# cafferychen777/flashdeconv

Hardware: AMD Instinct MI355X
Metric: spots/sec to convergence (1M x 2000 x 30) (higher is better)
Workload: dtype f64

## Files before the change

### flashdeconv_amd/_lib.py

```python
import ctypes
import os
import threading

import numpy as np

_HERE = os.path.dirname(os.path.abspath(__file__))
LIB_PATH = os.path.join(_HERE, "libfdx.so")

c_int = ctypes.c_int
c_i32 = ctypes.c_int32
c_i64 = ctypes.c_int64
c_double = ctypes.c_double
c_void_p = ctypes.c_void_p
c_size_t = ctypes.c_size_t
p_double = ctypes.POINTER(ctypes.c_double)
p_i64 = ctypes.POINTER(ctypes.c_int64)
p_i32 = ctypes.POINTER(ctypes.c_int32)


class FdxError(RuntimeError):
    """A libfdx call failed (message from fdx_last_error())."""


class SolveInfo(ctypes.Structure):
# ... 97 lines not shown
    "fdx_graph_shard_knn_dev": (c_int, [c_void_p, c_i64, c_i32, c_i32, c_i32, p_i64, c_i32, c_void_p, ctypes.POINTER(c_void_p)]),
    "fdx_graph_shard_status": (c_int, [c_void_p, p_i64, p_i64, p_i32, p_i32]),
    "fdx_graph_row_indices": (c_int, [c_void_p, c_i64, p_i32, c_i32, p_i32]),
    "fdx_graph_halo_info": (c_int, [c_void_p, p_i64, p_i32, p_i32]),
    "fdx_graph_send_indices_dev": (c_int, [c_void_p, c_void_p, c_void_p]),
    "fdx_prepare_dev": (c_int, [c_void_p, c_i32, c_i64, c_i32, c_i64, c_void_p, p_double, c_i32, p_i32, p_double, p_double,
                                c_i32, c_i32, c_i32, c_void_p, c_i64, c_void_p, p_double, p_double, c_void_p]),
    "fdx_init_beta_dev": (c_int, [c_void_p, c_i64, c_i64, c_i32, c_void_p]),
    "fdx_bcd_sweep_dev": (c_int, [c_void_p, c_void_p, c_i64, c_void_p, c_void_p, c_void_p, c_i64, c_i32, c_double, c_double,
                                  c_double, c_i32, c_void_p, c_void_p, c_void_p]),
    "fdx_bcd_fold_dev": (c_int, [c_void_p, c_void_p, c_i32, c_void_p]),
    "fdx_objective_partials_dev": (c_int, [c_void_p, c_void_p, c_i64, c_void_p, c_i64, c_void_p, c_i32, p_double, c_void_p]),
    "fdx_spot_diagnostics_dev": (c_int, [c_void_p, c_void_p, c_i64, c_void_p, c_i64, c_void_p, c_i32, c_i32, c_void_p, c_void_p,
                                         c_void_p]),
    "fdx_normalize_dev": (c_int, [c_void_p, c_i64, c_i64, c_i32, c_void_p, c_void_p, c_void_p]),
    "fdx_gene_moments_dev": (c_int, [c_void_p, c_i32, c_i64, c_i32, c_i64, p_double, p_double, c_void_p]),
    "fdx_gather_columns_dev": (c_int, [c_void_p, c_i32, c_i64, c_i32, c_i64, p_i32, c_i32, c_void_p, c_void_p]),
    "fdx_version": (c_int, []),
    "fdx_env_reload": (c_int, []),
    "fdx_env_switch": (ctypes.c_char_p, [c_i32, ctypes.POINTER(ctypes.c_char_p)]),
    "fdx_last_error": (ctypes.c_char_p, []),
    "fdx_device_count": (c_int, [ctypes.POINTER(c_int)]),
    "fdx_set_device": (c_int, [c_int]),
    "fdx_device_name": (c_int, [ctypes.c_char_p, c_int]),
    "fdx_malloc": (c_int, [ctypes.POINTER(c_void_p), c_size_t]),
    "fdx_free": (c_int, [c_void_p]),
    "fdx_trim": (c_int, []),
    "fdx_memcpy_h2d": (c_int, [c_void_p, c_void_p, c_size_t, c_void_p]),
    "fdx_memcpy_d2h": (c_int, [c_void_p, c_void_p, c_size_t, c_void_p]),
    "fdx_memset": (c_int, [c_void_p, c_int, c_size_t, c_void_p]),
# ... 451 lines not shown
```

### flashdeconv_amd/csrc/bcd_kernels.cpp

```cpp
#include <algorithm>

#include "bcd_device.h"

namespace fdx {

__global__ __launch_bounds__(256) void bcd_sweep_generic_kernel(BcdSweepArgs a, double* scratch, size_t sld) {
    const int lane = threadIdx.x & 63;
    const int wib = __builtin_amdgcn_readfirstlane(threadIdx.x >> 6);
    const int K = a.K;
    if (a.it > 0) {
        const double rc = fold_rel_change(a.stats + (size_t)(a.it - 1) * 128, lane);
        if (blockIdx.x == 0 && threadIdx.x == 0) a.rel_change[a.it - 1] = rc;
        if (rc < a.tol) return;
    }
    const int slice = xcd_remap(blockIdx.x, gridDim.x) * 4 + wib;
    if (slice >= a.n_slices) return;
    const int i = slice * 64 + lane;
    const bool active = i < a.n;
    const int ii = active ? i : a.n - 1;
    const size_t ld = (size_t)a.ld;
    const int w0 = a.slice_off[slice];
    const int w = a.slice_off[slice + 1] - w0;
    double* bb = scratch + (size_t)(slice * 64 + lane);
    const int* ell = a.ell + (size_t)w0 * 64 + lane;
// ... 310 lines not shown
        for (int A = 0; A < nblk; ++A)
            for (int B = A; B < nblk; ++B)
                hipLaunchKernelGGL(beta_quad_block_kernel, dim3(grid), dim3(256), 0, st, beta, ld, n, K, XtX, A * 4, B * 4, A == B ? 1.0 : 2.0,
                                   partials);
        FDX_CHECK_LAUNCH();
        return 0;
    }
#define FDX_BQ(T) case T: hipLaunchKernelGGL(beta_quad_kernel<T>, dim3(grid), dim3(256), 0, st, beta, ld, n, K, XtX, partials); break;
    switch (TT) { FDX_BQ(1) FDX_BQ(2) FDX_BQ(3) FDX_BQ(4) FDX_BQ(5) FDX_BQ(6) FDX_BQ(7) default: return fail(FDX_ERR_INVALID, "beta quad: K"); }
#undef FDX_BQ
    FDX_CHECK_LAUNCH();
    return 0;
}

int launch_bcd_objective_tiled(const BcdSweepArgs& a0, double* partials, hipStream_t st) {
    if (!a0.tiled || !sweep_instantiated(a0.K)) return 1;
    const int KC = a0.K < 8 ? a0.K : 8;
    if ((size_t)KC * (256 + a0.halo_max + 1) * sizeof(double) > 64 * 1024) return 1;
    BcdSweepArgs a = a0;
    a.objective = 1;
    a.rel_change = partials;
    a.it = 0;
    const bool hit = bcd_sweep_dispatch_part0(a, st) || bcd_sweep_dispatch_part1(a, st) || bcd_sweep_dispatch_part2(a, st) ||
                     bcd_sweep_dispatch_part3(a, st) || bcd_sweep_dispatch_part4(a, st) || bcd_sweep_dispatch_part5(a, st) ||
                     bcd_sweep_dispatch_part6(a, st) || bcd_sweep_dispatch_part7(a, st);
    if (!hit) return 1;
    FDX_CHECK_LAUNCH();
    return 0;
}

int launch_bcd_fold_last(const unsigned long long* stats, double* rel_change, int it, hipStream_t st) {
    hipLaunchKernelGGL(bcd_fold_last_kernel, dim3(1), dim3(64), 0, st, stats, rel_change, it);
    FDX_CHECK_LAUNCH();
// ... 5 lines not shown
```

### flashdeconv_amd/csrc/bcd_sweep_inst.cpp

```cpp
#include <algorithm>
#include <cstdlib>
#include "bcd_device.h"
#include "fdx_graph.h"

#ifndef FDX_PART
#error "compile with -DFDX_PART=<n> -DFDX_K_LO=<lo> -DFDX_K_HI=<hi>"
#endif

namespace fdx {

constexpr int sweep_chunk(int K) {
#ifdef FDX_KC_OVERRIDE
    return K < FDX_KC_OVERRIDE ? K : FDX_KC_OVERRIDE;
#endif
    return K < 8 ? K : K <= 29 ? 8 : K <= 33 ? 7 : K <= 37 ? 6 : K <= 41 ? 5 : K <= 45 ? 4 : K <= 49 ? 3 : K <= 51 ? 2 : K <= 64 ? 8 : K <= 72 ? 6 : K <= 88 ? 4 : K <= 96 ? 2 : 8;
}

template <int K, int KC>
__global__ __launch_bounds__(256) void bcd_sweep_kernel(
    const double* __restrict__ H, const double* __restrict__ XtX, const double* __restrict__ beta_in,
    double* __restrict__ beta_out, const int* __restrict__ ell_base, const int* __restrict__ slice_off,
    const int* __restrict__ deg, unsigned long long* __restrict__ stats, double* __restrict__ rel_change,
    const double lambda, const double rho, const double tol, const int ldh, const int ld_, const int n,
    const int n_slices, const int it) {
// ... 71 lines not shown
        atomicMax(s + 64 + slot, (unsigned long long)__double_as_longlong(amax));
    }
}

__device__ __forceinline__ const char __attribute__((address_space(1)))* plane_base(const double* p) {
    unsigned long long v = (unsigned long long)p;
    asm("" : "+s"(v));
    return (const char __attribute__((address_space(1)))*)v;
}

__device__ __forceinline__ unsigned lane_off(unsigned off) {
    asm("" : "+v"(off));
    return off;
}

#ifndef FDX_SWEEP_WPE
#define FDX_SWEEP_WPE 1
#endif
template <int K, int KC, bool OBJ, bool QUAD = true, bool INIT = false>
__global__ __launch_bounds__(256, ((OBJ && K > 40 && K <= 64) || (K > 64 && K <= 96)) ? 2 : (OBJ ? 1 : FDX_SWEEP_WPE)) void bcd_sweep_tiled_kernel(
    const double* __restrict__ H, const double* __restrict__ XtX, const double* __restrict__ beta_in,
    double* __restrict__ beta_out, const unsigned short* __restrict__ ell_local, const int* __restrict__ slice_off,
    const int* __restrict__ deg, const int* __restrict__ tile_halo, const int* __restrict__ tile_hcnt,
    unsigned long long* __restrict__ stats, double* __restrict__ rel_change, const double lambda, const double rho,
    const double tol, const int ldh, const int ld_, const int n, const int S, const int it,
    const int* __restrict__ tile_list, const double init_v, const int* __restrict__ send_head, const int4* __restrict__ send_ent,
    double* __restrict__ send_buf) {
    extern __shared__ __attribute__((aligned(16))) double lds[];
    const int tid = threadIdx.x;
    const int lane = tid & 63;
    const int tile = tile_list ? tile_list[xcd_remap(blockIdx.x, gridDim.x)] : xcd_remap(blockIdx.x, gridDim.x);
    const bool real = (tile * 256 + tid) < n;
    const int i = min(tile * 256 + tid, n - 1);
    const size_t ld = (size_t)ld_;
    const int slice = __builtin_amdgcn_readfirstlane(i >> 6);
    const int w0 = slice_off[slice];
    const int w = slice_off[slice + 1] - w0;
    const int Ht = tile_hcnt[tile];
    const int* halo = tile_halo + (size_t)tile * FDX_TILE_HALO_CAP;
    const int dg = deg[i];
    int hidx0 = halo[tid];
    if (!OBJ && it > 0) {
// ... 81 lines not shown
                if (!OBJ || QUAD) {
#pragma unroll
                    for (int j = 0; j + 1 < K; j += 2) {
                        r0 = fma(g[j], b[j], r0);
                        r1 = fma(g[j + 1], b[j + 1], r1);
                    }
                    if (K & 1) r0 = fma(g[K - 1], b[K - 1], r0);
                }
                const double gkk = (!OBJ || QUAD) ? g[k] : 0.0;
                const double old = b[k];
                if (OBJ) {
                    o_cross = fma(old, h, o_cross);
                    if (QUAD) o_quad = fma(old, r0 + r1, o_quad);
                    o_spat = fma(old, (double)dg * old - c[q], o_spat);
                    o_l1 += fabs(old);
                    asm volatile("" : "+v"(o_quad));
                } else {
                    const double res = (h - (r0 + r1) + gkk * old) + lam_eff * c[q];
                    const double den = gkk + lam_deg;
                    const double st = res > rho ? res - rho : (res < -rho ? res + rho : 0.0);
                    const double qv = fmax(0.0, st / den);
                    const double nw = (den > 1e-10) ? qv : 0.0;
                    dmax = fmax(dmax, fabs(nw - old));
                    amax = fmax(amax, fabs(old));
                    b[k] = nw;
                    __builtin_nontemporal_store(nw, (double __attribute__((address_space(1)))*)(plane_base(beta_out + k * ld) + lane_off(ioff)));
                }
            }
            if (kc + KC < K) {
#pragma unroll
                for (int t = 2 * q; t < 2 * q + 2; ++t) {
                    const int j = t < KC ? t : t - KC;
                    if (kc + KC + j < K) {
                        if (t < KC) { if (!INIT) hv[j] = PLANE_AT(beta_in + (kc + KC + j) * ld, hoff); }
                        else hreg[j] = __builtin_nontemporal_load(&PLANE_AT(H + (kc + KC + j) * (size_t)ldh, ioff));
                    }
                }
                __builtin_amdgcn_sched_barrier(0);
            }
        }
    }
    if (OBJ) {
        if (!real) { o_cross = o_quad = o_spat = o_l1 = 0.0; }
#pragma unroll
        for (int off = 32; off > 0; off >>= 1) {
            o_cross += __shfl_xor(o_cross, off, 64);
            o_quad += __shfl_xor(o_quad, off, 64);
            o_spat += __shfl_xor(o_spat, off, 64);
            o_l1 += __shfl_xor(o_l1, off, 64);
        }
        __syncthreads();
        if (lane == 0) { lds[(tid >> 6) * 4 + 0] = o_cross; lds[(tid >> 6) * 4 + 1] = o_quad; lds[(tid >> 6) * 4 + 2] = o_spat; lds[(tid >> 6) * 4 + 3] = o_l1; }
        __syncthreads();
        if (tid < 4) rel_change[(size_t)tile * 4 + tid] = ((lds[tid] + lds[4 + tid]) + lds[8 + tid]) + lds[12 + tid];
        return;
    }
    if (!OBJ && send_head != nullptr) {
// ... 15 lines not shown
        atomicMax(s + 64 + slot, (unsigned long long)__double_as_longlong(amax));
    }
}

template <int K>
static void launch_k(const BcdSweepArgs& a, hipStream_t st) {
    if (a.tiled) {
        constexpr int KC = sweep_chunk(K);
        const int S = 256 + a.halo_max + 1;
        const size_t lds = (size_t)KC * S * sizeof(double);
        if (lds <= 64 * 1024 && (long long)a.ld * 8 < (1LL << 32) && (long long)a.ldh * 8 < (1LL << 32)) {
            if (a.objective) {
                if constexpr (K > 64) {
                    hipLaunchKernelGGL((bcd_sweep_tiled_kernel<K, KC, true, false>), dim3(a.n_tiles), dim3(256), lds, st, a.H, a.XtX,
                                       a.beta_in, a.beta_out, a.ell_local, a.slice_off, a.deg, a.tile_halo, a.tile_hcnt,
                                       a.stats, a.rel_change, a.lambda, a.rho, a.tol, a.ldh, a.ld, a.n, S, a.it, nullptr, 0.0, a.send_head, a.send_ent, a.send_buf);
                } else {
                    hipLaunchKernelGGL((bcd_sweep_tiled_kernel<K, KC, true>), dim3(a.n_tiles), dim3(256), lds, st, a.H, a.XtX,
                                       a.beta_in, a.beta_out, a.ell_local, a.slice_off, a.deg, a.tile_halo, a.tile_hcnt,
                                       a.stats, a.rel_change, a.lambda, a.rho, a.tol, a.ldh, a.ld, a.n, S, a.it, nullptr, 0.0, a.send_head, a.send_ent, a.send_buf);
                }
            }
            else if (a.tile_list) {
                if (a.n_list > 0)
                    hipLaunchKernelGGL((bcd_sweep_tiled_kernel<K, KC, false>), dim3(a.n_list), dim3(256), lds, st, a.H, a.XtX,
                                       a.beta_in, a.beta_out, a.ell_local, a.slice_off, a.deg, a.tile_halo, a.tile_hcnt,
                                       a.stats, a.rel_change, a.lambda, a.rho, a.tol, a.ldh, a.ld, a.n, S, a.it, a.tile_list, 0.0, a.send_head, a.send_ent, a.send_buf);
            } else if (a.init_uniform != 0.0) {
                if constexpr (K <= 64) {
                    hipLaunchKernelGGL((bcd_sweep_tiled_kernel<K, KC, false, true, true>), dim3(a.n_tiles), dim3(256), lds, st, a.H, a.XtX,
                                       a.beta_in, a.beta_out, a.ell_local, a.slice_off, a.deg, a.tile_halo, a.tile_hcnt,
                                       a.stats, a.rel_change, a.lambda, a.rho, a.tol, a.ldh, a.ld, a.n, S, a.it, nullptr, a.init_uniform, a.send_head, a.send_ent, a.send_buf);
                }
            } else {
                hipLaunchKernelGGL((bcd_sweep_tiled_kernel<K, KC, false>), dim3(a.n_tiles), dim3(256), lds, st, a.H, a.XtX,
                                   a.beta_in, a.beta_out, a.ell_local, a.slice_off, a.deg, a.tile_halo, a.tile_hcnt,
                                   a.stats, a.rel_change, a.lambda, a.rho, a.tol, a.ldh, a.ld, a.n, S, a.it, nullptr, 0.0, a.send_head, a.send_ent, a.send_buf);
            }
            return;
        }
    }
    const int nblk = ceil_div(a.n_slices, 4);
    hipLaunchKernelGGL((bcd_sweep_kernel<K, sweep_chunk(K)>), dim3(nblk), dim3(256), 0, st, a.H, a.XtX, a.beta_in,
                       a.beta_out, a.ell, a.slice_off, a.deg, a.stats, a.rel_change, a.lambda, a.rho, a.tol, a.ldh,
                       a.ld, a.n, a.n_slices, a.it);
}

#ifndef FDX_K_STEP
#define FDX_K_STEP 1
#endif
template <int... Is>
static bool dispatch_range(const BcdSweepArgs& a, hipStream_t st, std::integer_sequence<int, Is...>) {
// ... 14 lines not shown
```

### flashdeconv_amd/csrc/capi_dev.cpp

```cpp
#include "fdx_env.h"
#include <algorithm>
#include <cmath>
#include <memory>
#include <vector>

#include "fdx_graph.h"
#include "fdx_internal.h"
#include "fdx_kernels.h"
#include "graph_build.h"
#include "prepare.h"
#include "sketch_plan.h"
#include "solver.h"

using namespace fdx;

extern "C" {

int fdx_graph_build_dev(const double* coords_dev, int64_t n, int32_t dim, int32_t method, int32_t k, double radius,
                        void* stream, fdx_graph** out) {
    PoolStream pool_stream((hipStream_t)stream);
    FDX_REQUIRE(out != nullptr, "fdx_graph_build_dev: null output");
    *out = nullptr;
    FDX_REQUIRE(n == 0 || coords_dev != nullptr, "fdx_graph_build_dev: null coords");
    fdx_graph* g = new fdx_graph();
// ... 297 lines not shown
    FDX_REQUIRE(g && beta_dev && H_dev && XtX_dev && out4_host, "fdx_objective_partials_dev: null argument");
    hipStream_t st = (hipStream_t)stream;
    PoolStream pool_stream(st);
    out4_host[0] = out4_host[1] = out4_host[2] = out4_host[3] = 0.0;
    if (g->n == 0) return 0;
    DevBuf part, out;
    const int nblk = objective_partials_count(g->n_slices);
    FDX_TRY(part.alloc((size_t)nblk * 4 * sizeof(double)));
    FDX_TRY(out.alloc(4 * sizeof(double)));
    FDX_TRY(solver_objective_partials(*g, beta_dev, ld, H_dev, ldh, XtX_dev, K, part.as<double>(), out.as<double>(), st));
    FDX_HIP(hipMemcpyAsync(out4_host, out.p, 4 * sizeof(double), hipMemcpyDeviceToHost, st));
    FDX_HIP(hipStreamSynchronize(st));
    return 0;
}

int fdx_spot_diagnostics_dev(const fdx_graph* g, const double* beta_dev, int64_t ld, const double* H_dev, int64_t ldh,
                             const double* XtX_dev, int32_t ldg, int32_t K, const double* row_sq_dev, double* out_dev,
                             void* stream) {
    FDX_TRY(fdx::graph_meta_sync(g));
    FDX_REQUIRE(g && beta_dev && H_dev && XtX_dev && row_sq_dev && out_dev, "fdx_spot_diagnostics_dev: null argument");
    FDX_REQUIRE(K >= 1 && ldg >= K, "fdx_spot_diagnostics_dev: K must be positive and ldg at least K");
    FDX_REQUIRE(ld >= g->n_total + 1, "fdx_spot_diagnostics_dev: ld must cover own + halo + zero row");
    FDX_REQUIRE(ldh >= g->n, "fdx_spot_diagnostics_dev: ldh must cover the own spots");
    if (g->n == 0) return 0;
    const int* perm = (g->identity_order || !g->perm.p || g->world_n > 0) ? nullptr : g->perm.as<int>();
    return launch_spot_diagnostics(beta_dev, ld, H_dev, ldh, XtX_dev, ldg, row_sq_dev, g->ell.as<int>(), g->slice_off.as<int>(),
                                   g->deg.as<int>(), perm, (int)g->n, g->n_slices, K, out_dev, (hipStream_t)stream);
}

int fdx_normalize_dev(const double* beta_dev, int64_t ld, int64_t n, int32_t K, double* beta_out_dev, double* prop_out_dev,
// ... 39 lines not shown
```

### flashdeconv_amd/csrc/comm.cpp

```cpp
#include "fdx_env.h"
#include <dlfcn.h>
#include <rccl/rccl.h>

#include <algorithm>
#include <cmath>
#include <condition_variable>
#include <cstdio>
#include <cstdlib>
#include <cstring>
#include <mutex>
#include <vector>

#include "fdx_graph.h"
#include "fdx_internal.h"
#include "fdx_kernels.h"
#include "graph_build.h"
#include "prepare.h"
#include "solver.h"

using namespace fdx;

namespace {

struct RcclApi {
// ... 471 lines not shown
    const double rho_eff = prm->rho_sparsity * diag_mean;
    info->lambda_used = lambda;
    info->rho_effective = rho_eff;

    const long long ld = round_up(g->n_total + 1, 64);
    FDX_TRY(dB0.alloc((size_t)KP * ld * sizeof(double)));
    FDX_TRY(dB1.alloc((size_t)KP * ld * sizeof(double)));
    int32_t which = 0;
    FDX_TRY(sharded_solve_impl(c, g, dH.as<double>(), ldh, XtX_dev, KP, K, lambda, rho_eff, prm->tol, prm->max_iter, dB0.as<double>(),
                               dB1.as<double>(), ld, &info->solve, rel_changes_out, &which, stream));
    const double* beta = which ? dB1.as<double>() : dB0.as<double>();
    shard_trace("loop returned");

    FDX_TRY(objp.alloc((size_t)std::max(objective_partials_count(g->n_slices), g->n_tiles) * 4 * sizeof(double)));
    FDX_TRY(dFin.alloc(8 * sizeof(double)));
    if (beta_out_dev || prop_out_dev) {
        FDX_HIP(hipEventRecord(c->ev_packed, st));
        FDX_HIP(hipStreamWaitEvent(c->side, c->ev_packed, 0));
        FDX_TRY(launch_normalize_export(beta, ld, nullptr, (int)n_own, g->n_slices, K, beta_out_dev, prop_out_dev, c->side));
        FDX_HIP(hipEventRecord(c->ev_halo, c->side));
    }
    FDX_TRY(solver_objective_partials(*g, beta, ld, dH.as<double>(), ldh, XtX_dev, KP, objp.as<double>(), dFin.as<double>(), st));
    if (job.evSum) FDX_TRY(job.evSum.wait_on(st));
    FDX_HIP(hipMemcpyAsync(dFin.as<double>() + 4, job.dSum.p, sizeof(double), hipMemcpyDeviceToDevice, st));
    FDX_TRY(allreduce(c, dFin.p, 5, false, st));
    FDX_HIP(hipMemcpyAsync(cnt_h, dFin.p, 5 * sizeof(double), hipMemcpyDeviceToHost, st));
    if (beta_out_dev || prop_out_dev) FDX_HIP(hipStreamWaitEvent(st, c->ev_halo, 0));
    FDX_HIP(hipStreamSynchronize(st));
    shard_trace("objective on the host");
    info->YtY = cnt_h[4];
    info->solve.final_objective = objective_from_sums(cnt_h, cnt_h[4], lambda, rho_eff);
    return 0;
}

static int sharded_solve_impl(fdx_comm* c, const fdx_graph* g, const double* H_dev, int64_t ldh, const double* XtX_dev, int32_t K,
                              int32_t K_real, double lambda, double rho_eff, double tol, int32_t max_iter, double* beta0_dev,
                              double* beta1_dev, int64_t ld, fdx_solve_info* info, double* rel_changes_out, int32_t* result_buffer,
                              void* stream) {
    FDX_REQUIRE(c && g && H_dev && XtX_dev && beta0_dev && beta1_dev && info && result_buffer, "fdx_sharded_solve_dev: null argument");
    FDX_TRY(fdx::graph_meta_sync(g));
    FDX_REQUIRE(K >= 1 && K_real >= 1 && K_real <= K && (sweep_instantiated(K) || K > FDX_MAX_K_FAST),
                "fdx_sharded_solve_dev: K must be 1..64, fdx_solver_padded_k of 65..96 cell types, or above 96");
// ... 142 lines not shown
```

### flashdeconv_amd/csrc/fdx_env.cpp

```cpp
#include "fdx_env.h"

#include <atomic>
#include <chrono>
#include <cstdio>
#include <cstdlib>
#include <cstring>
#include <deque>
#include <mutex>
#include <string>

#include "fdx_internal.h"

namespace fdx {
namespace {

struct Switch {
    const char* name;
    const char* what;
    std::atomic<const char*> value{nullptr};
};

Switch g_switches[] = {
    {"FDX_TRACE_HOST", "host time between the marked points of a fit / a graph build (stderr)"},
    {"FDX_DEBUG", "one-line reports of the routes taken (leverage route, ELL rebuilds)"},
// ... 6 lines not shown
    {"FDX_NO_OVERLAP", "sharded loop: one sweep launch per iteration, halo on the compute stream"},
    {"FDX_NO_FUSED", "two-kernel sketch -> H (scatter + contraction) instead of the tile kernel"},
    {"FDX_NO_TILE_WIDE", "no wide tile kernel (K > 32 / d > 704): the two-kernel path takes those shapes"},
    {"FDX_TILE_LOGV", "0: float64 log1p chain for float32 rows in the tile kernel"},
    {"FDX_SKETCH_GATHER", "gather form of the row sketch kernel"},
    {"FDX_GRAPH_SORT", "Morton order by a radix sort instead of by counting"},
    {"FDX_GRAPH_SYNC", "graph build completed inside the call (no deferred counts)"},
    {"FDX_GRAPH_TWO_ELL_KERNELS", "fill_ell + tile_halo as two kernels"},
    {"FDX_NO_FUSED_PACK", "sharded loop: halo_pack_kernel instead of the sweep writing the send staging"},
    {"FDX_LEV_ONE_WG", "leverage scores by the single-workgroup route"},
    {"FDX_KDTREE_HOST_QUERIES", "tie remedy: cKDTree queries on host threads instead of kd_query_kernel"},
    {"FDX_KDTREE_THREADS", "host threads of the restated cKDTree (build forks, host queries)"},
    {"FDX_KDTREE_PAR_DEPTH", "fork depth of the restated cKDTree build"},
    {"FDX_NO_PLAN_CACHE", "sketch plans / tile schedules rebuilt every fit (bench.py: cold_ms)"},
    {"FDX_NO_SIDE_STREAM", "everything on the caller's stream"},
    {"FDX_CSR_KEEP_CAP", "entries per wave of the fused CSR sketch's keep buffer (tests: rows that overflow it)"},
};
constexpr int kSwitches = sizeof(g_switches) / sizeof(g_switches[0]);
std::once_flag g_once;
std::mutex g_mu;
std::atomic<bool> g_trace_host{false};

const char* lookup(const char* name) {
    for (const Switch& s : g_switches)
        if (std::strcmp(s.name, name) == 0) return s.value.load(std::memory_order_acquire);
    return nullptr;
}

void load_all() {
    static std::deque<std::string>* const kept = new std::deque<std::string>();
// ... 49 lines not shown
```

### flashdeconv_amd/csrc/fdx_kernels.h

```cpp
#pragma once
#include <cstdlib>
#include <hip/hip_runtime.h>

#include <cstddef>
#include <cstdint>
#include <utility>
#include <initializer_list>

namespace fdx {

constexpr int FDX_MAX_K_FAST = 64;
constexpr int FDX_MAX_K_PAD = 96;
inline int solver_padded_K(int K) {
    if (K <= FDX_MAX_K_FAST || K > FDX_MAX_K_PAD) return K;
    for (int kp : {72, 80, 88, 96})
        if (K <= kp) return kp;
    return K;
}
inline bool sweep_instantiated(int K) { return K >= 1 && (K <= FDX_MAX_K_FAST || K == 72 || K == 80 || K == 88 || K == 96); }

struct BcdSweepArgs {
    const double* H;
    const double* XtX;
    const double* beta_in;
    double* beta_out;
    const int* ell;
    const int* slice_off;
    const int* deg;
    const unsigned short* ell_local = nullptr;
    const int* tile_halo = nullptr;
    const int* tile_hcnt = nullptr;
    int n_tiles = 0;
    int halo_max = 0;
    int tiled = 0;
    int objective = 0;
    int skip_quad = 0;
    const int* tile_list = nullptr;
    int n_list = 0;
    const int* send_head = nullptr;
    const int4* send_ent = nullptr;
    double* send_buf = nullptr;
    double init_uniform = 0.0;
    unsigned long long* stats;
    double* rel_change;
    double lambda;
    double rho;
    double tol;
    int ldh;
    int ld;
    int n;
    int n_slices;
// ... 100 lines not shown
```

### flashdeconv_amd/csrc/fit.cpp

```cpp
#include "fdx_env.h"
#include <algorithm>
#include <cstdio>
#include <cmath>
#include <cstdlib>
#include <memory>
#include <vector>

#include "fdx_graph.h"
#include "fdx_internal.h"
#include "fdx_kernels.h"
#include "graph_build.h"
#include "prepare.h"
#include "sketch_plan.h"
#include "solver.h"

using namespace fdx;

namespace {

int build_csc_from_tables(const int32_t* bucket, const double* weight, int G, int d, std::vector<long long>* col_ptr,
                          std::vector<int>* gene_idx, std::vector<double>* w) {
    col_ptr->assign((size_t)d + 1, 0);
    for (int g = 0; g < G; ++g) {
        FDX_REQUIRE(bucket[g] >= 0 && bucket[g] < d, "fit: bucket index out of range");
// ... 236 lines not shown
        FDX_REQUIRE(g != nullptr && g->n == n, "fdx_fit_dev: given graph does not match n");
    } else {
        FDX_REQUIRE(coords_dev != nullptr, "fdx_fit_dev: null coords");
        g = new fdx_graph();
        int rc = (prm->graph_method == FDX_GRAPH_KNN)
                     ? graph_build_knn(coords_dev, n, dim, prm->k_neighbors, g, st)
                     : graph_build_radius(coords_dev, n, dim, prm->radius, 0, n, g, st);
        if (rc) { delete g; return rc; }
        *graph_inout = g;
    }
    if (g->meta_pending && g->meta_event && g->meta_stream != st) FDX_HIP(hipStreamWaitEvent(st, g->meta_event, 0));
    FDX_TRY(t_graph.record(st));

    const long long ld = round_up(n + 1, 64);
    const int KP = solver_padded_K(K);
    DevBuf dB0, dB1, dH, dSum;
    XSide x;
    YTables tables;
    RowsToH rows;
    struct SideDrain { hipStream_t s = nullptr; ~SideDrain() { if (s) (void)hipStreamSynchronize(s); } } side_drain;
    struct AbortDrain { hipStream_t s; bool armed = true; ~AbortDrain() { if (armed) (void)hipStreamSynchronize(s); } } abort_drain{st};
    Event evInit, evG;
    hipStream_t side = fdx::env("FDX_NO_SIDE_STREAM") ? nullptr : library_side_stream();
    if (side == st) side = nullptr;
    const hipStream_t xs = side ? side : st;
    if (side) side_drain.s = side;
    for (int g_ = 0; g_ < G; ++g_) FDX_REQUIRE(bucket[g_] >= 0 && bucket[g_] < d, "fit: bucket index out of range");
    double* Gh = (double*)pinned_scratch(0, (size_t)K * K * sizeof(double));
    FDX_REQUIRE(Gh != nullptr, "fit: pinned host buffer");
    const bool beta0_virtual = side && KP == K && K <= FDX_MAX_K_FAST && prm->max_iter > 0 && !prm->verbose && !fdx::env("FDX_NO_INIT_SWEEP");
    {
// ... 70 lines not shown
    const double diag_mean = xtx_diag_mean(Gh, K);
    const double lambda = prm->lambda_auto ? auto_lambda(diag_mean, (double)g->nnz / (double)n) : prm->lambda_spatial;

    SolveProblem p;
    p.graph = g; p.H = dH.as<double>(); p.ldh = ld; p.XtX = XtX_dev;
    p.beta[0] = dB0.as<double>(); p.beta[1] = dB1.as<double>(); p.ld = ld; p.K = KP; p.K_real = K; p.YtY = prm->verbose ? *YtY_h : 0.0;
    p.lambda = lambda; p.rho_eff = prm->rho_sparsity * diag_mean; p.max_iter = prm->max_iter; p.tol = prm->tol;
    p.verbose = prm->verbose;
    p.compute_objective = prm->verbose ? 1 : 0;
    SolveResult r;
    if (evInit) {
        p.init_beta = 0;
        p.beta0_virtual = beta0_virtual ? 1 : 0;
        FDX_TRY(evInit.wait_on(st));
    }
    FDX_TRY(solver_run(p, &r, st));
    Event evSolved, evExported;
    if ((beta_out_dev || prop_out_dev) && !prm->verbose && side) {
        FDX_TRY(evSolved.record(st));
        FDX_TRY(evSolved.wait_on(side));
        FDX_TRY(launch_normalize_export(p.beta[r.result_buffer], ld, row_map, (int)n, g->n_slices, K, beta_out_dev,
                                        prop_out_dev, side));
        FDX_TRY(evExported.record(side));
    }
    if (!prm->verbose) {
        DevBuf objp, objo;
        FDX_TRY(objp.alloc((size_t)std::max(objective_partials_count(g->n_slices), g->n_tiles) * 4 * sizeof(double)));
        FDX_TRY(objo.alloc(4 * sizeof(double)));
        if (prm->max_iter == 0) FDX_HIP(hipStreamSynchronize(st));
        if (evY) FDX_TRY(evY.sync());
        FDX_TRY(solver_objective(*g, p.beta[r.result_buffer], ld, p.H, ld, p.XtX, KP, *YtY_h, lambda, p.rho_eff, objp.as<double>(),
                                 objo.as<double>(), &r.final_objective, st));
    }
    FDX_TRY(t_solved.record(st));
    if (evExported) FDX_TRY(evExported.wait_on(st));
    else if (beta_out_dev || prop_out_dev)
        FDX_TRY(launch_normalize_export(p.beta[r.result_buffer], ld, row_map, (int)n, g->n_slices, K, beta_out_dev,
                                        prop_out_dev, st));
    Event t_diag0(true), t_diag1(true);
    if (prm->spot_diag_out_dev) {
        FDX_TRY(t_diag0.record(st));
        FDX_TRY(launch_spot_diagnostics(p.beta[r.result_buffer], ld, p.H, ld, XtX_dev, KP, rows.dRowSq.as<double>(), g->ell.as<int>(),
                                        g->slice_off.as<int>(), g->deg.as<int>(), row_map, (int)n, g->n_slices, K,
                                        prm->spot_diag_out_dev, st));
        FDX_TRY(t_diag1.record(st));
    }
    FDX_TRY(t_end.record(st));
    FDX_HIP(hipStreamSynchronize(st));
    abort_drain.armed = false;

    info->solve.converged = r.converged;
    info->solve.n_iterations = r.n_iterations;
    info->solve.final_objective = r.final_objective;
    info->solve.final_change = r.final_change;
    info->solve.n_objectives = (int32_t)r.objectives.size();
    info->solve.sweep_ms = r.sweep_ms;
    info->lambda_used = lambda;
    info->rho_effective = p.rho_eff;
    info->YtY = *YtY_h;
    info->nnz = g->nnz;
    info->graph_ms = t_graph.ms_since(t_begin.e);
    info->sketch_ms = rows.fused ? eS1.ms_since(eS0.e) : rows.sketch_ms;
    info->gram_ms = rows.gram_ms;
    const bool from_build = g->begin_event && g->begin_stream == st && prm->graph_method == FDX_GRAPH_GIVEN;
// ... 100 lines not shown
```

### flashdeconv_amd/csrc/solver.cpp

```cpp
#include "fdx_env.h"
#include "solver.h"

#include <algorithm>
#include <cmath>
#include <cstdlib>
#include <vector>

namespace fdx {

__global__ void fill_beta_kernel(double* b, long long ld, long long n_fill, int K, double value, int K_planes) {
    const long long i = blockIdx.x * (long long)blockDim.x + threadIdx.x;
    if (i >= ld) return;
    const double v = (i < n_fill) ? value : 0.0;
    for (int k = 0; k < K; ++k) b[(size_t)k * ld + i] = v;
    for (int k = K; k < K_planes; ++k) b[(size_t)k * ld + i] = 0.0;
}

__global__ void pad_square_kernel(const double* __restrict__ A, int K, double* __restrict__ B, int KP) {
    const int e = blockIdx.x * blockDim.x + threadIdx.x;
    if (e >= KP * KP) return;
    const int i = e / KP, j = e - i * KP;
    B[e] = (i < K && j < K) ? A[i * K + j] : 0.0;
}

// ... 74 lines not shown
        FDX_TRY(launch_objective_partials(beta, ld, H, ldh, XtX, g.ell.as<int>(), g.slice_off.as<int>(), g.deg.as<int>(),
                                          (int)g.n, g.n_slices, K, scratch_partials, st, skip_quad));
        if (skip_quad) FDX_TRY(launch_beta_quad(beta, ld, g.n, K, XtX, scratch_partials, nblk, st));
    }
    return launch_sum_partials(scratch_partials, nblk, out4_dev, 4, 4, st);
}

int solver_objective(const fdx_graph& g, const double* beta, long long ld, const double* H, long long ldh,
                     const double* XtX, int K, double YtY, double lambda, double rho_eff, double* scratch_partials,
                     double* scratch_out4, double* obj_host, hipStream_t st) {
    FDX_TRY(solver_objective_partials(g, beta, ld, H, ldh, XtX, K, scratch_partials, scratch_out4, st));
    double r[4];
    FDX_HIP(hipMemcpyAsync(r, scratch_out4, sizeof(r), hipMemcpyDeviceToHost, st));
    FDX_HIP(hipStreamSynchronize(st));
    *obj_host = objective_from_sums(r, YtY, lambda, rho_eff);
    return 0;
}

int SweepStats::init(int max_iter, hipStream_t st) {
    const size_t iters = (size_t)std::max(max_iter, 1);
    const size_t stats_bytes = iters * 128 * sizeof(unsigned long long);
    FDX_TRY(block.alloc(stats_bytes + iters * sizeof(double)));
    FDX_HIP(hipMemsetAsync(block.p, 0, block.bytes, st));
    stats = block.as<unsigned long long>();
    rel_change = reinterpret_cast<double*>(static_cast<char*>(block.p) + stats_bytes);
    return 0;
}

int solver_loop(const SweepStats& s, int max_iter, double tol, int first_chunk, int n_ahead,
                const std::function<int(int, bool)>& queue_iteration, LoopResult* res, hipStream_t st) {
// ... 116 lines not shown
```

### flashdeconv_amd/csrc/solver.h

```cpp
#pragma once
#include <functional>
#include <vector>

#include "fdx_graph.h"
#include "fdx_internal.h"
#include "fdx_kernels.h"

namespace fdx {

struct SolveProblem {
    const fdx_graph* graph = nullptr;
    const double* H = nullptr;
    long long ldh = 0;
    const double* XtX = nullptr;
    double* beta[2] = {nullptr, nullptr};
    long long ld = 0;
    int K = 0;
    int K_real = 0;
    double YtY = 0.0;
    double lambda = 0.0;
    double rho_eff = 0.0;
    int max_iter = 100;
    double tol = 1e-4;
    int verbose = 0;
// ... 12 lines not shown
    double sweep_ms = 0.0;
    std::vector<int> objective_iters;
    std::vector<double> objectives;
    std::vector<double> rel_changes;
};

int solver_init_beta(double* beta, long long ld, long long n_fill, int K, hipStream_t st, int K_planes = 0);
int solver_pad_square(const double* A, int K, double* B, int KP, hipStream_t st);
int solver_zero_pad(double* b, long long ld, long long n_used, int K, hipStream_t st);
int solver_objective_partials(const fdx_graph& g, const double* beta, long long ld, const double* H, long long ldh,
                              const double* XtX, int K, double* scratch_partials, double* out4_dev, hipStream_t st);
int solver_objective(const fdx_graph& g, const double* beta, long long ld, const double* H, long long ldh,
                     const double* XtX, int K, double YtY, double lambda, double rho_eff, double* scratch_partials,
                     double* scratch_out4, double* obj_host, hipStream_t st);
int solver_run(const SolveProblem& p, SolveResult* res, hipStream_t st);

BcdSweepArgs sweep_args_for_graph(const fdx_graph& g, bool honour_no_tiled);
int sweep_scratch_prepare(const double* XtX, int K, int n_slices, DevBuf* scratch, size_t* scratch_ld, hipStream_t st);
double xtx_diag_mean(const double* XtX_host, int K);
double auto_lambda(double diag_mean, double mean_degree);
inline double objective_from_sums(const double* r4, double YtY, double lambda, double rho_eff) {
    return 0.5 * (YtY - 2.0 * r4[0] + r4[1]) + 0.5 * lambda * r4[2] + rho_eff * r4[3];
}

struct SweepStats {
    DevBuf block;
    unsigned long long* stats = nullptr;
    double* rel_change = nullptr;
    int init(int max_iter, hipStream_t st);
};
// ... 11 lines not shown
```

### include/fdx.h

```cpp
#ifndef FDX_H
#define FDX_H

#include <stddef.h>
#include <stdint.h>

#ifdef __cplusplus
extern "C" {
#endif

#define FDX_OK 0
#define FDX_ERR_INVALID (-1)
#define FDX_ERR_HIP (-2)
#define FDX_ERR_UNSUPPORTED (-3)
#define FDX_ERR_INTERNAL (-4)

#define FDX_F32 0
#define FDX_F64 1

#define FDX_PRE_RAW 0
#define FDX_PRE_LOG_CPM 1
#define FDX_PRE_LOG_CPM_SPARSE 2
#define FDX_PRE_F64_MATH 0x100

int fdx_version(void);
// ... 230 lines not shown
                    double* XtX_out_host, double* YtY_partial_out, void* stream);
int fdx_prepare_csr_dev(const fdx_csr_view* Y, const int32_t* gene_idx, int32_t G, const double* X, int32_t K,
                        const int32_t* bucket, const double* weight_y, const double* weight_x, int32_t d, int32_t mode_y,
                        int32_t mode_x, double* H_out_dev, int64_t ldh, double* XtX_out_dev, double* XtX_out_host,
                        double* YtY_partial_out, void* stream);
int fdx_init_beta_dev(double* beta_dev, int64_t ld, int64_t n_fill, int32_t K, void* stream);
int fdx_bcd_sweep_dev(const fdx_graph* g, const double* H_dev, int64_t ldh, const double* XtX_dev, const double* beta_in,
                      double* beta_out, int64_t ld, int32_t K, double lambda, double rho_eff, double tol, int32_t it,
                      void* stats_dev, double* rel_change_dev, void* stream);
int fdx_bcd_fold_dev(void* stats_dev, double* rel_change_dev, int32_t it, void* stream);
int fdx_objective_partials_dev(const fdx_graph* g, const double* beta_dev, int64_t ld, const double* H_dev, int64_t ldh,
                               const double* XtX_dev, int32_t K, double* out4_host, void* stream);
int fdx_spot_diagnostics_dev(const fdx_graph* g, const double* beta_dev, int64_t ld, const double* H_dev, int64_t ldh,
                             const double* XtX_dev, int32_t ldg, int32_t K, const double* row_sq_dev, double* out_dev,
                             void* stream);
int fdx_normalize_dev(const double* beta_dev, int64_t ld, int64_t n, int32_t K, double* beta_out_dev, double* prop_out_dev,
                      void* stream);

typedef struct fdx_comm fdx_comm;
typedef struct fdx_local_world fdx_local_world;
int fdx_comm_unique_id(void* id_out_128);
int fdx_comm_init(const void* id_128, int32_t rank, int32_t world, fdx_comm** out);
int fdx_local_world_create(int32_t world, fdx_local_world** out);
int fdx_comm_init_loopback(int32_t rank, int32_t world, fdx_comm** out);
int fdx_local_world_destroy(fdx_local_world* w);
int fdx_comm_init_local(fdx_local_world* w, int32_t rank, fdx_comm** out);
int fdx_comm_destroy(fdx_comm* comm);
int fdx_comm_info(const fdx_comm* comm, int32_t* rank, int32_t* world);
int fdx_comm_rccl_count(const fdx_comm* comm, int32_t* count);
int fdx_comm_allreduce_sum_dev(fdx_comm* comm, double* buf_dev, int32_t count, void* stream);
// ... 34 lines not shown
```

Before: 239.8 million.

## Fuse final objective pass with beta/proportion export in one tiled traversal

Adds a fused finish path where the tiled objective sweep kernel also writes the normalized proportions and beta to the output buffers. It stages rows through LDS for coalesced nontemporal stores. This replaces a separate normalize/export kernel plus the objective kernel, so beta is read from memory once instead of twice. The host sync and readback of the objective sums are deferred to the end of the fit, which adds LDS pressure and complexity in the objective kernel.

```diff
diff --git a/flashdeconv_amd/_lib.py b/flashdeconv_amd/_lib.py
--- a/flashdeconv_amd/_lib.py
+++ b/flashdeconv_amd/_lib.py
@@ -135,6 +135,7 @@
     "fdx_spot_diagnostics_dev": (c_int, [c_void_p, c_void_p, c_i64, c_void_p, c_i64, c_void_p, c_i32, c_i32, c_void_p, c_void_p,
                                          c_void_p]),
     "fdx_normalize_dev": (c_int, [c_void_p, c_i64, c_i64, c_i32, c_void_p, c_void_p, c_void_p]),
+    "fdx_finish_dev": (c_int, [c_void_p, c_void_p, c_i64, c_void_p, c_i64, c_void_p, c_i32, c_void_p, c_void_p, p_double, c_void_p]),
     "fdx_gene_moments_dev": (c_int, [c_void_p, c_i32, c_i64, c_i32, c_i64, p_double, p_double, c_void_p]),
     "fdx_gather_columns_dev": (c_int, [c_void_p, c_i32, c_i64, c_i32, c_i64, p_i32, c_i32, c_void_p, c_void_p]),
     "fdx_version": (c_int, []),
diff --git a/flashdeconv_amd/csrc/bcd_kernels.cpp b/flashdeconv_amd/csrc/bcd_kernels.cpp
--- a/flashdeconv_amd/csrc/bcd_kernels.cpp
+++ b/flashdeconv_amd/csrc/bcd_kernels.cpp
@@ -348,9 +348,7 @@
 }
 
 int launch_bcd_objective_tiled(const BcdSweepArgs& a0, double* partials, hipStream_t st) {
-    if (!a0.tiled || !sweep_instantiated(a0.K)) return 1;
-    const int KC = a0.K < 8 ? a0.K : 8;
-    if ((size_t)KC * (256 + a0.halo_max + 1) * sizeof(double) > 64 * 1024) return 1;
+    if (!bcd_sweep_uses_tiles(a0)) return 1;
     BcdSweepArgs a = a0;
     a.objective = 1;
     a.rel_change = partials;
diff --git a/flashdeconv_amd/csrc/bcd_sweep_inst.cpp b/flashdeconv_amd/csrc/bcd_sweep_inst.cpp
--- a/flashdeconv_amd/csrc/bcd_sweep_inst.cpp
+++ b/flashdeconv_amd/csrc/bcd_sweep_inst.cpp
@@ -109,6 +109,50 @@
     return off;
 }
 
+typedef double double2_t __attribute__((ext_vector_type(2)));
+constexpr int export_rows(int K) { return K <= 15 ? 64 : K <= 31 ? 32 : 16; }
+constexpr size_t export_lds_bytes(int K) { return (size_t)4 * export_rows(K) * (K | 1) * sizeof(double); }
+
+template <int K, bool PROP>
+__device__ __forceinline__ void export_staged(const double (&b)[K], const double s, const double den, double* tile, const int lane,
+                                              const int orow, double* __restrict__ out, const bool wide) {
+    constexpr int R = export_rows(K), Ks = K | 1;
+    const double inv_K = 1.0 / (double)K;
+#pragma unroll
+    for (int r0 = 0; r0 < 64; r0 += R) {
+        if ((lane & ~(R - 1)) == r0) {
+            double* t = tile + (lane - r0) * Ks;
+#pragma unroll
+            for (int k = 0; k < K; ++k) t[k] = PROP ? ((s == 0.0) ? inv_K : b[k] / den) : b[k];
+        }
+        __builtin_amdgcn_wave_barrier();
+        if ((K & 1) == 0 && wide) {
+            constexpr int total = R * K / 2;
+#pragma unroll 1
+            for (int f0 = 0; f0 < total; f0 += 64) {
+                const int f = f0 + lane;
+                const int e = 2 * min(f, total - 1);
+                const int sp = e / K, k = e - sp * K;
+                const int row = __shfl(orow, r0 + sp, 64);
+                const double2_t v = {tile[sp * Ks + k], tile[sp * Ks + k + 1]};
+                if (f < total && row >= 0) __builtin_nontemporal_store(v, (double2_t*)(out + (size_t)row * K + k));
+            }
+        } else {
+            constexpr int total = R * K;
+#pragma unroll 1
+            for (int f0 = 0; f0 < total; f0 += 64) {
+                const int f = f0 + lane;
+                const int e = min(f, total - 1);
+                const int sp = e / K, k = e - sp * K;
+                const int row = __shfl(orow, r0 + sp, 64);
+                const double v = tile[sp * Ks + k];
+                if (f < total && row >= 0) __builtin_nontemporal_store(v, out + (size_t)row * K + k);
+            }
+        }
+        __builtin_amdgcn_wave_barrier();
+    }
+}
+
 #ifndef FDX_SWEEP_WPE
 #define FDX_SWEEP_WPE 1
 #endif
@@ -120,7 +164,7 @@
     unsigned long long* __restrict__ stats, double* __restrict__ rel_change, const double lambda, const double rho,
     const double tol, const int ldh, const int ld_, const int n, const int S, const int it,
     const int* __restrict__ tile_list, const double init_v, const int* __restrict__ send_head, const int4* __restrict__ send_ent,
-    double* __restrict__ send_buf) {
+    double* __restrict__ send_buf, double* __restrict__ exp_beta, double* __restrict__ exp_prop, const int* __restrict__ exp_perm) {
     extern __shared__ __attribute__((aligned(16))) double lds[];
     const int tid = threadIdx.x;
     const int lane = tid & 63;
@@ -232,7 +276,7 @@
                     if (QUAD) o_quad = fma(old, r0 + r1, o_quad);
                     o_spat = fma(old, (double)dg * old - c[q], o_spat);
                     o_l1 += fabs(old);
-                    asm volatile("" : "+v"(o_quad));
+                    asm volatile("" : "+v"(o_quad), "+v"(o_cross), "+v"(o_spat), "+v"(o_l1));
                 } else {
                     const double res = (h - (r0 + r1) + gkk * old) + lam_eff * c[q];
                     const double den = gkk + lam_deg;
@@ -259,6 +303,19 @@
         }
     }
     if (OBJ) {
+        if constexpr (K <= FDX_MAX_K_FAST) {
+            if (exp_beta != nullptr || exp_prop != nullptr) {
+                const int orow = real ? (exp_perm ? exp_perm[i] : i) : -1;
+                double* wtile = lds + (tid >> 6) * (export_rows(K) * (K | 1));
+                if (exp_beta) export_staged<K, false>(b, 0.0, 1.0, wtile, lane, orow, exp_beta, ((size_t)exp_beta & 15) == 0);
+                if (exp_prop) {
+                    double s = 0.0;
+#pragma unroll
+                    for (int k = 0; k < K; ++k) s += b[k];
+                    export_staged<K, true>(b, s, fmax(s, 1e-10), wtile, lane, orow, exp_prop, ((size_t)exp_prop & 15) == 0);
+                }
+            }
+        }
         if (!real) { o_cross = o_quad = o_spat = o_l1 = 0.0; }
 #pragma unroll
         for (int off = 32; off > 0; off >>= 1) {
@@ -304,28 +361,29 @@
                 if constexpr (K > 64) {
                     hipLaunchKernelGGL((bcd_sweep_tiled_kernel<K, KC, true, false>), dim3(a.n_tiles), dim3(256), lds, st, a.H, a.XtX,
                                        a.beta_in, a.beta_out, a.ell_local, a.slice_off, a.deg, a.tile_halo, a.tile_hcnt,
-                                       a.stats, a.rel_change, a.lambda, a.rho, a.tol, a.ldh, a.ld, a.n, S, a.it, nullptr, 0.0, a.send_head, a.send_ent, a.send_buf);
+                                       a.stats, a.rel_change, a.lambda, a.rho, a.tol, a.ldh, a.ld, a.n, S, a.it, nullptr, 0.0, a.send_head, a.send_ent, a.send_buf, nullptr, nullptr, nullptr);
                 } else {
-                    hipLaunchKernelGGL((bcd_sweep_tiled_kernel<K, KC, true>), dim3(a.n_tiles), dim3(256), lds, st, a.H, a.XtX,
+                    const size_t lds_o = std::max(lds, (a.exp_beta || a.exp_prop) ? export_lds_bytes(K) : (size_t)0);
+                    hipLaunchKernelGGL((bcd_sweep_tiled_kernel<K, KC, true>), dim3(a.n_tiles), dim3(256), lds_o, st, a.H, a.XtX,
                                        a.beta_in, a.beta_out, a.ell_local, a.slice_off, a.deg, a.tile_halo, a.tile_hcnt,
-                                       a.stats, a.rel_change, a.lambda, a.rho, a.tol, a.ldh, a.ld, a.n, S, a.it, nullptr, 0.0, a.send_head, a.send_ent, a.send_buf);
+                                       a.stats, a.rel_change, a.lambda, a.rho, a.tol, a.ldh, a.ld, a.n, S, a.it, nullptr, 0.0, a.send_head, a.send_ent, a.send_buf, a.exp_beta, a.exp_prop, a.exp_perm);
                 }
             }
             else if (a.tile_list) {
                 if (a.n_list > 0)
                     hipLaunchKernelGGL((bcd_sweep_tiled_kernel<K, KC, false>), dim3(a.n_list), dim3(256), lds, st, a.H, a.XtX,
                                        a.beta_in, a.beta_out, a.ell_local, a.slice_off, a.deg, a.tile_halo, a.tile_hcnt,
-                                       a.stats, a.rel_change, a.lambda, a.rho, a.tol, a.ldh, a.ld, a.n, S, a.it, a.tile_list, 0.0, a.send_head, a.send_ent, a.send_buf);
+                                       a.stats, a.rel_change, a.lambda, a.rho, a.tol, a.ldh, a.ld, a.n, S, a.it, a.tile_list, 0.0, a.send_head, a.send_ent, a.send_buf, a.exp_beta, a.exp_prop, a.exp_perm);
             } else if (a.init_uniform != 0.0) {
                 if constexpr (K <= 64) {
                     hipLaunchKernelGGL((bcd_sweep_tiled_kernel<K, KC, false, true, true>), dim3(a.n_tiles), dim3(256), lds, st, a.H, a.XtX,
                                        a.beta_in, a.beta_out, a.ell_local, a.slice_off, a.deg, a.tile_halo, a.tile_hcnt,
-                                       a.stats, a.rel_change, a.lambda, a.rho, a.tol, a.ldh, a.ld, a.n, S, a.it, nullptr, a.init_uniform, a.send_head, a.send_ent, a.send_buf);
+                                       a.stats, a.rel_change, a.lambda, a.rho, a.tol, a.ldh, a.ld, a.n, S, a.it, nullptr, a.init_uniform, a.send_head, a.send_ent, a.send_buf, a.exp_beta, a.exp_prop, a.exp_perm);
                 }
             } else {
                 hipLaunchKernelGGL((bcd_sweep_tiled_kernel<K, KC, false>), dim3(a.n_tiles), dim3(256), lds, st, a.H, a.XtX,
                                    a.beta_in, a.beta_out, a.ell_local, a.slice_off, a.deg, a.tile_halo, a.tile_hcnt,
-                                   a.stats, a.rel_change, a.lambda, a.rho, a.tol, a.ldh, a.ld, a.n, S, a.it, nullptr, 0.0, a.send_head, a.send_ent, a.send_buf);
+                                   a.stats, a.rel_change, a.lambda, a.rho, a.tol, a.ldh, a.ld, a.n, S, a.it, nullptr, 0.0, a.send_head, a.send_ent, a.send_buf, a.exp_beta, a.exp_prop, a.exp_perm);
             }
             return;
         }
diff --git a/flashdeconv_amd/csrc/capi_dev.cpp b/flashdeconv_amd/csrc/capi_dev.cpp
--- a/flashdeconv_amd/csrc/capi_dev.cpp
+++ b/flashdeconv_amd/csrc/capi_dev.cpp
@@ -335,6 +335,39 @@
     return 0;
 }
 
+int fdx_finish_dev(const fdx_graph* g, const double* beta_dev, int64_t ld, const double* H_dev, int64_t ldh, const double* XtX_dev,
+                   int32_t K, double* beta_out_dev, double* prop_out_dev, double* out4_host, void* stream) {
+    FDX_TRY(fdx::graph_meta_sync(g));
+    FDX_REQUIRE(g && beta_dev && H_dev && XtX_dev && out4_host, "fdx_finish_dev: null argument");
+    FDX_REQUIRE(K >= 1, "fdx_finish_dev: K must be positive");
+    FDX_REQUIRE(ld >= g->n_total + 1, "fdx_finish_dev: ld must cover own + halo + zero row");
+    FDX_REQUIRE(ldh >= g->n, "fdx_finish_dev: ldh must cover the own spots");
+    hipStream_t st = (hipStream_t)stream;
+    PoolStream pool_stream(st);
+    out4_host[0] = out4_host[1] = out4_host[2] = out4_host[3] = 0.0;
+    if (g->n == 0) return 0;
+    const int* perm = (g->identity_order || !g->perm.p || g->world_n > 0) ? nullptr : g->perm.as<int>();
+    DevBuf part, out;
+    FDX_TRY(part.alloc((size_t)std::max(objective_partials_count(g->n_slices), g->n_tiles) * 4 * sizeof(double)));
+    FDX_TRY(out.alloc(4 * sizeof(double)));
+    double* pin = (double*)pinned_scratch(7, 4 * sizeof(double));
+    FDX_REQUIRE(pin != nullptr, "fdx_finish_dev: pinned host buffer");
+    const int rc = solver_finish(*g, beta_dev, ld, H_dev, ldh, XtX_dev, K, perm, beta_out_dev, prop_out_dev, part.as<double>(),
+                                 out.as<double>(), pin, st);
+    if (rc < 0) { (void)hipStreamSynchronize(st); return rc; }
+    if (rc != 0) {
+        int rc2 = solver_objective_partials(*g, beta_dev, ld, H_dev, ldh, XtX_dev, K, part.as<double>(), out.as<double>(), st);
+        if (!rc2 && (beta_out_dev || prop_out_dev))
+            rc2 = launch_normalize_export(beta_dev, ld, perm, (int)g->n, g->n_slices, K, beta_out_dev, prop_out_dev, st);
+        if (!rc2 && hipMemcpyAsync(pin, out.p, 4 * sizeof(double), hipMemcpyDeviceToHost, st) != hipSuccess)
+            rc2 = fdx::fail(FDX_ERR_HIP, "fdx_finish_dev: copy of the sums");
+        if (rc2) { (void)hipStreamSynchronize(st); return rc2; }
+    }
+    FDX_HIP(hipStreamSynchronize(st));
+    for (int o = 0; o < 4; ++o) out4_host[o] = pin[o];
+    return 0;
+}
+
 int fdx_spot_diagnostics_dev(const fdx_graph* g, const double* beta_dev, int64_t ld, const double* H_dev, int64_t ldh,
                              const double* XtX_dev, int32_t ldg, int32_t K, const double* row_sq_dev, double* out_dev,
                              void* stream) {
diff --git a/flashdeconv_amd/csrc/comm.cpp b/flashdeconv_amd/csrc/comm.cpp
--- a/flashdeconv_amd/csrc/comm.cpp
+++ b/flashdeconv_amd/csrc/comm.cpp
@@ -509,18 +509,24 @@
 
     FDX_TRY(objp.alloc((size_t)std::max(objective_partials_count(g->n_slices), g->n_tiles) * 4 * sizeof(double)));
     FDX_TRY(dFin.alloc(8 * sizeof(double)));
-    if (beta_out_dev || prop_out_dev) {
+    const int fused = KP == K ? solver_finish(*g, beta, ld, dH.as<double>(), ldh, XtX_dev, K, nullptr, beta_out_dev, prop_out_dev,
+                                              objp.as<double>(), dFin.as<double>(), nullptr, st)
+                              : 1;
+    if (fused < 0) return fused;
+    const bool side_export = fused != 0 && (beta_out_dev || prop_out_dev);
+    if (side_export) {
         FDX_HIP(hipEventRecord(c->ev_packed, st));
         FDX_HIP(hipStreamWaitEvent(c->side, c->ev_packed, 0));
         FDX_TRY(launch_normalize_export(beta, ld, nullptr, (int)n_own, g->n_slices, K, beta_out_dev, prop_out_dev, c->side));
         FDX_HIP(hipEventRecord(c->ev_halo, c->side));
     }
-    FDX_TRY(solver_objective_partials(*g, beta, ld, dH.as<double>(), ldh, XtX_dev, KP, objp.as<double>(), dFin.as<double>(), st));
+    if (fused != 0)
+        FDX_TRY(solver_objective_partials(*g, beta, ld, dH.as<double>(), ldh, XtX_dev, KP, objp.as<double>(), dFin.as<double>(), st));
     if (job.evSum) FDX_TRY(job.evSum.wait_on(st));
     FDX_HIP(hipMemcpyAsync(dFin.as<double>() + 4, job.dSum.p, sizeof(double), hipMemcpyDeviceToDevice, st));
     FDX_TRY(allreduce(c, dFin.p, 5, false, st));
     FDX_HIP(hipMemcpyAsync(cnt_h, dFin.p, 5 * sizeof(double), hipMemcpyDeviceToHost, st));
-    if (beta_out_dev || prop_out_dev) FDX_HIP(hipStreamWaitEvent(st, c->ev_halo, 0));
+    if (side_export) FDX_HIP(hipStreamWaitEvent(st, c->ev_halo, 0));
     FDX_HIP(hipStreamSynchronize(st));
     shard_trace("objective on the host");
     info->YtY = cnt_h[4];
diff --git a/flashdeconv_amd/csrc/fdx_env.cpp b/flashdeconv_amd/csrc/fdx_env.cpp
--- a/flashdeconv_amd/csrc/fdx_env.cpp
+++ b/flashdeconv_amd/csrc/fdx_env.cpp
@@ -44,6 +44,7 @@
     {"FDX_KDTREE_PAR_DEPTH", "fork depth of the restated cKDTree build"},
     {"FDX_NO_PLAN_CACHE", "sketch plans / tile schedules rebuilt every fit (bench.py: cold_ms)"},
     {"FDX_NO_SIDE_STREAM", "everything on the caller's stream"},
+    {"FDX_NO_FUSED_FINISH", "objective pass and export as two kernels instead of one traversal (bit-identical: tests)"},
     {"FDX_CSR_KEEP_CAP", "entries per wave of the fused CSR sketch's keep buffer (tests: rows that overflow it)"},
 };
 constexpr int kSwitches = sizeof(g_switches) / sizeof(g_switches[0]);
diff --git a/flashdeconv_amd/csrc/fdx_kernels.h b/flashdeconv_amd/csrc/fdx_kernels.h
--- a/flashdeconv_amd/csrc/fdx_kernels.h
+++ b/flashdeconv_amd/csrc/fdx_kernels.h
@@ -35,6 +35,9 @@
     int tiled = 0;
     int objective = 0;
     int skip_quad = 0;
+    double* exp_beta = nullptr;
+    double* exp_prop = nullptr;
+    const int* exp_perm = nullptr;
     const int* tile_list = nullptr;
     int n_list = 0;
     const int* send_head = nullptr;
diff --git a/flashdeconv_amd/csrc/fit.cpp b/flashdeconv_amd/csrc/fit.cpp
--- a/flashdeconv_amd/csrc/fit.cpp
+++ b/flashdeconv_amd/csrc/fit.cpp
@@ -274,7 +274,7 @@
 
     const long long ld = round_up(n + 1, 64);
     const int KP = solver_padded_K(K);
-    DevBuf dB0, dB1, dH, dSum;
+    DevBuf dB0, dB1, dH, dSum, objp, objo;
     XSide x;
     YTables tables;
     RowsToH rows;
@@ -375,29 +375,40 @@
         p.beta0_virtual = beta0_virtual ? 1 : 0;
         FDX_TRY(evInit.wait_on(st));
     }
-    FDX_TRY(solver_run(p, &r, st));
-    Event evSolved, evExported;
-    if ((beta_out_dev || prop_out_dev) && !prm->verbose && side) {
-        FDX_TRY(evSolved.record(st));
-        FDX_TRY(evSolved.wait_on(side));
-        FDX_TRY(launch_normalize_export(p.beta[r.result_buffer], ld, row_map, (int)n, g->n_slices, K, beta_out_dev,
-                                        prop_out_dev, side));
-        FDX_TRY(evExported.record(side));
-    }
+    double* sums_h = nullptr;
     if (!prm->verbose) {
-        DevBuf objp, objo;
         FDX_TRY(objp.alloc((size_t)std::max(objective_partials_count(g->n_slices), g->n_tiles) * 4 * sizeof(double)));
         FDX_TRY(objo.alloc(4 * sizeof(double)));
-        if (prm->max_iter == 0) FDX_HIP(hipStreamSynchronize(st));
-        if (evY) FDX_TRY(evY.sync());
-        FDX_TRY(solver_objective(*g, p.beta[r.result_buffer], ld, p.H, ld, p.XtX, KP, *YtY_h, lambda, p.rho_eff, objp.as<double>(),
-                                 objo.as<double>(), &r.final_objective, st));
-    }
+        sums_h = (double*)pinned_scratch(6, 4 * sizeof(double));
+        FDX_REQUIRE(sums_h != nullptr, "fit: pinned host buffer");
+    }
+    FDX_TRY(solver_run(p, &r, st));
     FDX_TRY(t_solved.record(st));
-    if (evExported) FDX_TRY(evExported.wait_on(st));
-    else if (beta_out_dev || prop_out_dev)
-        FDX_TRY(launch_normalize_export(p.beta[r.result_buffer], ld, row_map, (int)n, g->n_slices, K, beta_out_dev,
-                                        prop_out_dev, st));
+    int fused = 1;
+    if (!prm->verbose && KP == K)
+        fused = solver_finish(*g, p.beta[r.result_buffer], ld, p.H, ld, p.XtX, K, row_map, beta_out_dev, prop_out_dev, objp.as<double>(),
+                              objo.as<double>(), sums_h, st);
+    if (fused < 0) return fused;
+    if (fused != 0) {
+        Event evSolved, evExported;
+        if ((beta_out_dev || prop_out_dev) && !prm->verbose && side) {
+            FDX_TRY(evSolved.record(st));
+            FDX_TRY(evSolved.wait_on(side));
+            FDX_TRY(launch_normalize_export(p.beta[r.result_buffer], ld, row_map, (int)n, g->n_slices, K, beta_out_dev,
+                                            prop_out_dev, side));
+            FDX_TRY(evExported.record(side));
+        }
+        if (!prm->verbose) {
+            if (prm->max_iter == 0) FDX_HIP(hipStreamSynchronize(st));
+            if (evY) FDX_TRY(evY.sync());
+            FDX_TRY(solver_objective(*g, p.beta[r.result_buffer], ld, p.H, ld, p.XtX, KP, *YtY_h, lambda, p.rho_eff, objp.as<double>(),
+                                     objo.as<double>(), &r.final_objective, st));
+        }
+        if (evExported) FDX_TRY(evExported.wait_on(st));
+        else if (beta_out_dev || prop_out_dev)
+            FDX_TRY(launch_normalize_export(p.beta[r.result_buffer], ld, row_map, (int)n, g->n_slices, K, beta_out_dev,
+                                            prop_out_dev, st));
+    }
     Event t_diag0(true), t_diag1(true);
     if (prm->spot_diag_out_dev) {
         FDX_TRY(t_diag0.record(st));
@@ -409,6 +420,10 @@
     FDX_TRY(t_end.record(st));
     FDX_HIP(hipStreamSynchronize(st));
     abort_drain.armed = false;
+    if (fused == 0) {
+        if (evY) FDX_TRY(evY.sync());
+        r.final_objective = objective_from_sums(sums_h, *YtY_h, lambda, p.rho_eff);
+    }
 
     info->solve.converged = r.converged;
     info->solve.n_iterations = r.n_iterations;
diff --git a/flashdeconv_amd/csrc/solver.cpp b/flashdeconv_amd/csrc/solver.cpp
--- a/flashdeconv_amd/csrc/solver.cpp
+++ b/flashdeconv_amd/csrc/solver.cpp
@@ -112,6 +112,21 @@
     FDX_HIP(hipMemcpyAsync(r, scratch_out4, sizeof(r), hipMemcpyDeviceToHost, st));
     FDX_HIP(hipStreamSynchronize(st));
     *obj_host = objective_from_sums(r, YtY, lambda, rho_eff);
+    return 0;
+}
+
+int solver_finish(const fdx_graph& g, const double* beta, long long ld, const double* H, long long ldh, const double* XtX, int K,
+                  const int* perm, double* beta_out, double* prop_out, double* scratch_partials, double* out4_dev,
+                  double* out4_pinned, hipStream_t st) {
+    if (fdx::env("FDX_NO_FUSED_FINISH") || K > FDX_MAX_K_FAST || g.n <= 0) return 1;
+    BcdSweepArgs a = sweep_args_for_graph(g, true);
+    if (!a.tiled) return 1;
+    a.H = H; a.XtX = XtX; a.beta_in = beta; a.ldh = (int)ldh; a.ld = (int)ld; a.K = K;
+    a.exp_beta = beta_out; a.exp_prop = prop_out; a.exp_perm = perm;
+    const int rc = launch_bcd_objective_tiled(a, scratch_partials, st);
+    if (rc != 0) return rc;
+    FDX_TRY(launch_sum_partials(scratch_partials, g.n_tiles, out4_dev, 4, 4, st));
+    if (out4_pinned) FDX_HIP(hipMemcpyAsync(out4_pinned, out4_dev, 4 * sizeof(double), hipMemcpyDeviceToHost, st));
     return 0;
 }
 
diff --git a/flashdeconv_amd/csrc/solver.h b/flashdeconv_amd/csrc/solver.h
--- a/flashdeconv_amd/csrc/solver.h
+++ b/flashdeconv_amd/csrc/solver.h
@@ -50,6 +50,9 @@
                      const double* XtX, int K, double YtY, double lambda, double rho_eff, double* scratch_partials,
                      double* scratch_out4, double* obj_host, hipStream_t st);
 int solver_run(const SolveProblem& p, SolveResult* res, hipStream_t st);
+int solver_finish(const fdx_graph& g, const double* beta, long long ld, const double* H, long long ldh, const double* XtX, int K,
+                  const int* perm, double* beta_out, double* prop_out, double* scratch_partials, double* out4_dev,
+                  double* out4_pinned, hipStream_t st);
 
 BcdSweepArgs sweep_args_for_graph(const fdx_graph& g, bool honour_no_tiled);
 int sweep_scratch_prepare(const double* XtX, int K, int n_slices, DevBuf* scratch, size_t* scratch_ld, hipStream_t st);
diff --git a/include/fdx.h b/include/fdx.h
--- a/include/fdx.h
+++ b/include/fdx.h
@@ -268,6 +268,8 @@
 int fdx_spot_diagnostics_dev(const fdx_graph* g, const double* beta_dev, int64_t ld, const double* H_dev, int64_t ldh,
                              const double* XtX_dev, int32_t ldg, int32_t K, const double* row_sq_dev, double* out_dev,
                              void* stream);
+int fdx_finish_dev(const fdx_graph* g, const double* beta_dev, int64_t ld, const double* H_dev, int64_t ldh, const double* XtX_dev,
+                   int32_t K, double* beta_out_dev, double* prop_out_dev, double* out4_host, void* stream);
 int fdx_normalize_dev(const double* beta_dev, int64_t ld, int64_t n, int32_t K, double* beta_out_dev, double* prop_out_dev,
                       void* stream);
 
```

Result: slower. 236.1 million (-1.6%).
